# AkshayThiru/incentive-design-mpc

Hardware: AMD Instinct MI355X
Metric: LoMPC QP solves/sec (higher is better)
Workload: dtype f64

## Files before the change

### incentive-design-mpc_amd/csrc/lompc_plan.hip

```cpp
#include <hip/hip_ext.h>
#include <hip/hip_runtime.h>
#include <stdint.h>
#include <string.h>

#include <algorithm>
#include <chrono>
#include <cmath>
#include <cstdlib>
#include <map>
#include <mutex>
#include <type_traits>
#include <utility>

#include "lompc_ctx.hpp"
#include "lompc_loopstep.hpp"
#include "lompc_wave.hpp"

#ifdef LOMPC_STAMPS
#ifdef LOMPC_STAMPS_RT
#define __builtin_amdgcn_s_memtime __builtin_amdgcn_s_memrealtime
#endif
__device__ long long g_stamps[65536 * 8];
__device__ long long g_wstart[32768 * 8];
__device__ unsigned long long g_lstamps[64 * 16];
#define LQ_WSTART()                                                                              \
  do {                                                                                           \
    const long long t__ = __builtin_amdgcn_s_memtime();                                          \
    if ((threadIdx.x & 63) == 0 && blockIdx.x < 32768) g_wstart[blockIdx.x * 8 + (threadIdx.x >> 6)] = t__; \
  } while (0)
#define LQ_STAMPE(k)                                                                        \
  do {                                                                                      \
    const long long t__ = __builtin_amdgcn_s_memtime();                                     \
    if (threadIdx.x == 0 && blockIdx.x < 32768) g_stamps[(32768 + blockIdx.x) * 8 + (k)] = t__; \
  } while (0)
#define LQ_STAMPW(k)                                                                        \
  do {                                                                                      \
    asm volatile("s_waitcnt vmcnt(0)" ::: "memory");                                        \
    LQ_STAMPE(k);                                                                           \
  } while (0)
#define LQ_STAMP(k)                                                                         \
  do {                                                                                      \
    const long long t__ = __builtin_amdgcn_s_memtime();                                     \
    if ((threadIdx.x & 63) == 0 && blk < 65536) g_stamps[blk * 8 + (k)] = t__;              \
  } while (0)
#else
#define LQ_STAMP(k)
#define LQ_STAMPE(k)
#define LQ_STAMPW(k)
#define LQ_WSTART()
#endif

#ifndef EVAL_WAVES
#define EVAL_WAVES 8
#endif
#ifndef EVAL_RU
#define EVAL_RU 2
#endif
#ifndef EVAL_MIN_WAVES
#define EVAL_MIN_WAVES ((2 * EVAL_WAVES + 3) / 4)
#endif
#define EVAL_EVS (64 * EVAL_WAVES)
#ifndef EVAL_PASSES
#define EVAL_PASSES 2
#endif
#define EVAL_MAXB (EVAL_EVS * EVAL_PASSES)
#ifndef LQ_PIECE_CAP
#define LQ_PIECE_CAP 128
#endif
#define LQ_GMAX 1024
#ifndef LQ_EVAL_OUT_AFTER_ROWS
#define LQ_EVAL_OUT_AFTER_ROWS 1
#endif
#ifndef LQ_DIAG_NOLOOKUP
#define LQ_DIAG_NOLOOKUP 0
#endif
#ifndef LQ_DIAG_NOROWLDS
#define LQ_DIAG_NOROWLDS 0
#endif
#ifndef LQ_STEP_CELLS
#define LQ_STEP_CELLS 4
#endif
#ifndef LQ_STEP_PRIO
#define LQ_STEP_PRIO 1
#endif
#ifndef LQ_WARM_FP64
#define LQ_WARM_FP64 1
#endif
#define LQ_DROP_OFF 0x7fff0000

namespace {

typedef unsigned int lq_v4u __attribute__((ext_vector_type(4)));
typedef unsigned int lq_v2u __attribute__((ext_vector_type(2)));

#ifndef LQ_ROW_AUX
#define LQ_ROW_AUX 16
#endif
__device__ __forceinline__ void st_wt16(__amdgpu_buffer_rsrc_t rs, int off, double x, double y) {
  __builtin_amdgcn_raw_buffer_store_b128(__builtin_bit_cast(lq_v4u, make_double2(x, y)), rs, off, 0, LQ_ROW_AUX);
}
__device__ __forceinline__ void st_wt8b(__amdgpu_buffer_rsrc_t rs, int off, double x) {
  __builtin_amdgcn_raw_buffer_store_b64(__builtin_bit_cast(lq_v2u, x), rs, off, 0, LQ_ROW_AUX);
}
__device__ __forceinline__ void st_wt8(double* p, double v) {
  __hip_atomic_store(reinterpret_cast<unsigned long long*>(p), __builtin_bit_cast(unsigned long long, v),
                     __ATOMIC_RELAXED, __HIP_MEMORY_SCOPE_AGENT);
}

#ifndef LQ_EV_PLAIN
#define LQ_EV_PLAIN 0
#endif
__device__ __forceinline__ void st_ev8(double* p, double v) {
  if (LQ_EV_PLAIN) *p = v;
  else st_wt8(p, v);
}

__device__ __forceinline__ void st_wt4(int* p, int v) {
  __hip_atomic_store(p, v, __ATOMIC_RELAXED, __HIP_MEMORY_SCOPE_AGENT);
}

__host__ __device__ constexpr int eval_row_stride(int N) { return N + 1; }
__device__ __forceinline__ int cfx(const int k, const int j) {
  return k * 8 + ((((j >> 1) ^ (k >> 2)) & 3) << 1) + (j & 1);
}
static_assert((LQ_PPL & (LQ_PPL - 1)) == 0, "k_eval's piece-end transpose needs a power-of-two LQ_PPL");

#ifndef LQ_EVALS_STAGER
#define LQ_EVALS_STAGER 0
#endif
#ifndef LQ_EVALS_CAP
#define LQ_EVALS_CAP 64
#endif
#ifndef LQ_STG_CHUNK
#define LQ_STG_CHUNK 8
#endif
#define LQ_EVALS_RW 7
#define LQ_EVALS_MAXB (LQ_EVALS_RW * 64 * EVAL_PASSES)

struct CTab {
  double2* ab;
  double* cf;
  double* ge;
  double* lo;
  int* cnt;
  int* pre;
  int* meta;
};
__host__ __device__ inline size_t ctab_bytes(int N, int G, int capc) {
  const size_t b = (size_t)(capc + 2) * eval_row_stride(N) * 16 + (size_t)capc * 64 + (size_t)(capc + 8) * 8 +
                   (size_t)G * 16 + 16;
  return (b + 15) & ~(size_t)15;
}
__device__ __forceinline__ CTab ctab_at(char* base, int N, int G, int capc) {
  CTab t;
  t.ab = reinterpret_cast<double2*>(base);
  t.cf = reinterpret_cast<double*>(base + (size_t)(capc + 2) * eval_row_stride(N) * 16);
  t.ge = t.cf + (size_t)capc * 8;
  t.lo = t.ge + capc + 8;
  t.cnt = reinterpret_cast<int*>(t.lo + G);
  t.pre = t.cnt + G;
  t.meta = t.pre + G;
  return t;
}
inline size_t evals_st_lds(int N, int G, int capc) {
  return 2 * ctab_bytes(N, G, capc) + (size_t)2 * EVAL_WAVES * (N + 8) * sizeof(double);
}

__device__ __forceinline__ double clampw(double x, double wmax) { return fmin(fmax(x, 0.0), wmax); }

typedef const __attribute__((address_space(4))) QPConst QPConstK;
__device__ __forceinline__ const QPConst& set_consts(const QPConst* qd, const CtxEnds& ce, int s) {
  s = __builtin_amdgcn_readfirstlane(s);
  int k = 0;
#pragma unroll
  for (int j = 0; j + 1 < LQ_PLAN_MAX_CTX; ++j) k += s >= ce.end[j] ? 1 : 0;
  QPConstK* p = (QPConstK*)(uintptr_t)qd + k;
  return *(const QPConst*)p;
}

struct WindowArgs {
  const QPConst* qd;
  CtxEnds ce;
  const int4* blk;
  const int* blk_prefix;
  const double* gamma;
  unsigned long long* acc;
  double* window;
  int S, nblk;
};

__device__ __forceinline__ void window_store(double* window, int s, double ym, bool any, double lo, double hi) {
  const double mg = 1e-7 * ym;
  double wlo = 0.0, whi = ym;
  if (any) {
    wlo = fmin(fmax(lo - mg, 0.0), ym);
    whi = fmin(fmax(hi + mg, wlo + mg), ym);
    if (!(whi > wlo)) wlo = fmax(whi - 2.0 * mg, 0.0);
  }
  window[2 * s] = wlo;
  window[2 * s + 1] = whi;
}

__global__ __launch_bounds__(256) void k_plan_window(WindowArgs a) {
  __shared__ double smin[4], smax[4];
  __shared__ int last;
  if ((int)blockIdx.x == a.nblk) {
    for (int s = threadIdx.x; s < a.S; s += 256)
      if (a.blk_prefix[s + 1] == a.blk_prefix[s]) {
        int k = 0;
        for (int j = 0; j + 1 < LQ_PLAN_MAX_CTX; ++j) k += s >= a.ce.end[j] ? 1 : 0;
        a.window[2 * s] = 0.0;
        a.window[2 * s + 1] = a.qd[k].y_max;
      }
    return;
  }
  const int4 bk = a.blk[blockIdx.x];
// ... 602 lines not shown
    const bool is_max = c >= SN && (c - SN) % LOMPC_SET_STATS == LOMPC_STAT_MAX_ERR;
    double v = recv[c];
    for (int k = 1; k < nranks; ++k) {
      const double x = recv[(size_t)k * L + c];
      v = is_max ? fmax(v, x) : v + x;
    }
    if (c < SN) {
      if (set_sum_w) set_sum_w[c] = v;
    } else if (set_stats) {
      set_stats[c - SN] = v;
    }
  }
}

struct CombineRunsArgs {
  const double* recv;
  int nranks, n, S, N, run0, last;
  double* set_sum_w;
  double* set_stats;
  int64_t sw_stride, st_stride;
};
__global__ __launch_bounds__(256) void k_combine_runs(CombineRunsArgs a) {
  const int SN = a.S * a.N, L = a.S * (a.N + LOMPC_SET_STATS);
  const int64_t tot = (int64_t)a.n * L;
  for (int64_t e = (int64_t)blockIdx.x * 256 + threadIdx.x; e < tot; e += (int64_t)gridDim.x * 256) {
    const int r = (int)(e / L), c = (int)(e - (int64_t)r * L), j = a.run0 + r;
    const bool is_max = c >= SN && (c - SN) % LOMPC_SET_STATS == LOMPC_STAT_MAX_ERR;
    double v = a.recv[(size_t)r * L + c];
    for (int k = 1; k < a.nranks; ++k) {
      const double x = a.recv[((size_t)k * a.n + r) * L + c];
      v = is_max ? fmax(v, x) : v + x;
    }
    if (c < SN) {
      if (a.set_sum_w && (a.sw_stride || j == a.last)) a.set_sum_w[(size_t)j * a.sw_stride + c] = v;
    } else if (a.set_stats && (a.st_stride || j == a.last)) {
      a.set_stats[(size_t)j * a.st_stride + c - SN] = v;
    }
  }
}

__global__ __launch_bounds__(256) void k_chain_price(const QPConst* __restrict__ q, CtxEnds ce, int nctx, int N,
                                                     const double* __restrict__ prev, const double* __restrict__ sum_w,
                                                     const double* __restrict__ stats,
                                                     const double* __restrict__ target, double step,
                                                     double* __restrict__ next) {
  const int s = blockIdx.x;
  int k = 0;
  while (k + 1 < nctx && s >= ce.end[k]) ++k;
  const double th = q[k].theta, wm = q[k].w_max, qs = q[k].q_scale;
  const double n = stats[(size_t)s * LOMPC_SET_STATS + LOMPC_STAT_COUNT];
  for (int i = threadIdx.x; i < 3 * N; i += blockDim.x) {
    const int seg = i / N, t = i - seg * N;
    const double x = prev[(size_t)s * 3 * N + i];
    double v = x;
    if (n > 0) {
      const double wb = sum_w[(size_t)s * N + t] / n, wr = target[(size_t)s * N + t];
      const double g = seg == 0 ? th * (wb - wr) : (seg == 1 ? th * ((wm - wb) - (wm - wr)) : qs * (wb * wb - wr * wr));
      v = fmax(0.0, x + step * g);
    }
    next[(size_t)s * 3 * N + i] = v;
  }
}

struct RunOff {
  int64_t tab = 0;
  int rec = 0;
  int64_t ev = 0;
  const double* lmbd = nullptr;
  const double* lmbd_r = nullptr;
  bool launder = false;
  bool gamma_lds = false;
  bool nostage = false;
  bool pipelined = false;
  bool first = false;
  int buf = 0;
};

__device__ __forceinline__ void stage_compact(const EvalArgs& a, const int s, const int64_t tab, const CTab T,
                                           const int N, const int G, const int capc, const int lane) {
  const int64_t cb = tab + (int64_t)s * G;
  int cn = 0;
  double cl = 0.0;
  if (lane < G) {
    cn = min(max(ld_t<false>(a.t_cnt + cb + lane), 0), LQ_PPL);
    cl = ld_t<false>(a.t_lo + cb + lane);
  }
  int incl = cn;
#pragma unroll
  for (int d = 1; d < 64; d <<= 1) {
    const int y = __shfl_up(incl, d, 64);
    if (lane >= d) incl += y;
  }
  const bool fit = incl <= capc;
  const int ends = fit ? incl : 0x7fffffff;
  const int pre = incl - cn;
  int np = fit ? incl : 0, mx = fit ? cn : 0;
#pragma unroll
  for (int d = 32; d >= 1; d >>= 1) {
    np = max(np, __shfl_xor(np, d, 64));
    mx = max(mx, __shfl_xor(mx, d, 64));
  }
  if (lane < G) {
    T.cnt[lane] = fit ? cn : 0;
    T.pre[lane] = pre;
    T.lo[lane] = cl;
  }
  if (lane == 0) {
    T.meta[0] = mx;
    T.meta[1] = np;
  }
  const int NS = eval_row_stride(N);
  const size_t sb = (size_t)cb * LQ_PPL;
  for (int p0 = 0; p0 < np; p0 += LQ_STG_CHUNK) {
    double2 v[LQ_STG_CHUNK];
    int sl = 0;
#pragma unroll
    for (int u = 0; u < LQ_STG_CHUNK; ++u) {
      const int p = p0 + u;
      const int c = __popcll(__ballot(lane < G && ends <= p));
      const int slot = c * LQ_PPL + p - __builtin_amdgcn_readlane(pre, min(c, 63));
      if (lane == u) sl = slot;
      const double2* src = lane < N ? a.t_ab + (sb + slot) * N + lane
                                    : reinterpret_cast<const double2*>(a.t_cf + (sb + slot) * 8) + (lane - N);
      v[u] = p < np && lane < N + 4 ? ld_t<false>(src) : make_double2(0.0, 0.0);
    }
    const double vg = lane < LQ_STG_CHUNK && p0 + lane < np ? ld_t<false>(a.t_ge + sb + sl) : 0.0;
#pragma unroll
    for (int u = 0; u < LQ_STG_CHUNK; ++u) {
      const int p = p0 + u;
      if (p < np) {
        if (lane < N) T.ab[p * NS + ((N & 1) ? lane : (lane & 1) * (N >> 1) + (lane >> 1))] = v[u];
        else if (lane < N + 4) *reinterpret_cast<double2*>(T.cf + cfx(p, 2 * (lane - N))) = v[u];
      }
    }
    if (lane < LQ_STG_CHUNK && p0 + lane < np) T.ge[p0 + lane] = vg;
  }
}

template <int NT = 0, bool CLOSE = false, bool STG = false>
__device__ __forceinline__ void eval_block(const EvalArgs& a, const int blk, const FinalArgs* fr = nullptr,
                                           const RunOff ro = RunOff{}) {
  static_assert(!(STG && CLOSE), "the staged form has no in-launch closing");
  extern __shared__ __attribute__((aligned(16))) double2 s_dyn[];
  __shared__ double s_g[EVAL_MAXB];
  __shared__ int s_k[EVAL_MAXB];
  __shared__ double s_accw[EVAL_WAVES][LOMPC_MAX_N];
  __shared__ double s_red[EVAL_WAVES][8];
  __shared__ int s_fc[EVAL_WAVES];
  __shared__ int s_last;
  __shared__ int s_mx;
  __shared__ int s_done;
  int tid_ = (int)threadIdx.x;
  if (ro.launder) asm volatile("" : "+v"(tid_));
  const int tid = tid_, lane = tid & 63, wv = tid >> 6;
  const int4 info = a.blk[blk];
  const int rb = ro.rec + blk;
  double* const aw = a.w ? a.w + ro.ev * (NT ? NT : a.N) : nullptr;
  double* const acost = a.cost ? a.cost + ro.ev : nullptr;
  double* const aw0 = a.w0 ? a.w0 + ro.ev : nullptr;
  int8_t* const astatus = a.status ? a.status + ro.ev : nullptr;
  const int s = info.x, start = info.y, end = info.z;
  const int sg_per = STG ? (end - start + LQ_EVALS_RW - 1) / LQ_EVALS_RW : 0;
  const int sg0 = STG ? wv * sg_per : 0;
  const int sgn = STG ? max(0, min(sg_per, end - start - sg0)) : 0;
  auto brow = [&](const int h) { return STG ? sg0 + 64 * h + lane : tid + EVAL_EVS * h; };
  auto bact = [&](const int h) { return STG ? 64 * h + lane < sgn : start + tid + EVAL_EVS * h < end; };
  LQ_STAMPW(6);
  int G_ = a.G, cap_ = a.cap;
  if (ro.launder) asm volatile("" : "+s"(G_), "+s"(cap_));
  const int N = NT ? NT : a.N, G = G_;
  const int cap = cap_;
  const int ZK = cap;
  const int ZD = cap + 1;
  const bool psum = !CLOSE && !STG && ro.pipelined && a.piece_sums && !aw;
  LQ_STAMPE(0);
  LQ_WSTART();
  const int NS = eval_row_stride(N);
  auto abx = [&](const int k, const int t) { return k * NS + ((N & 1) ? t : (t & 1) * (N >> 1) + (t >> 1)); };
  double2* s_ab = s_dyn;
  double* s_cf = reinterpret_cast<double*>(s_ab + (size_t)(cap + 2) * NS);
  double* s_ge = s_cf + (size_t)cap * 8;
  double* s_lo = s_ge + cap;
  int* s_cnt = reinterpret_cast<int*>(s_lo + G);
  int* s_pre = nullptr;
  int stg_meta[2] = {0, 0};
  if constexpr (STG) {
    const CTab T = ctab_at(reinterpret_cast<char*>(s_dyn) + (size_t)ro.buf * ctab_bytes(N, G, cap), N, G, cap);
    s_ab = T.ab;
    s_cf = T.cf;
    s_ge = T.ge;
    s_lo = T.lo;
    s_cnt = T.cnt;
    s_pre = T.pre;
    stg_meta[0] = T.meta[0];
    stg_meta[1] = T.meta[1];
  }
  unsigned long long* s_pf = reinterpret_cast<unsigned long long*>(s_cnt + ((G + 1) & ~1));
  int* s_pn = reinterpret_cast<int*>(s_pf + cap + 2);
  const int np = STG ? stg_meta[1] : min(G * LQ_PPL, cap);
  const int Gs = STG ? G : np / LQ_PPL;
  constexpr int CPW = (LQ_PIECE_CAP / LQ_PPL + EVAL_WAVES - 1) / EVAL_WAVES;
  constexpr int UA = ((NT ? NT : LOMPC_MAX_N) * LQ_PPL + 63) / 64;
  int wc = 0;
  if (!STG && lane < CPW && wv + EVAL_WAVES * lane < Gs)
    wc = ld_t<false>(a.t_cnt + ro.tab + (size_t)s * G + wv + EVAL_WAVES * lane);
  double gh[EVAL_PASSES];
#pragma unroll
  for (int h = 0; h < EVAL_PASSES; ++h) {
    const int i = start + brow(h);
    gh[h] = ro.gamma_lds ? s_g[brow(h)] : bact(h) ? a.gamma[i] : 0.0;
  }
  const QPConst& q = set_consts(a.qd, a.ce, s);
  double wlo = a.window[2 * s], whi = a.window[2 * s + 1];
  const double* __restrict__ L = (ro.lmbd ? ro.lmbd : a.lmbd) + (size_t)s * 3 * N;
  double l0[3] = {L[0], L[N], L[2 * N]};
  double lr = (ro.lmbd_r ? ro.lmbd_r : a.lmbd_r)[s];
  const int64_t cb = ro.tab + (int64_t)s * G;
  const size_t sb = (size_t)cb * LQ_PPL;
  if (ro.pipelined && ro.first && tid == 0) s_done = 0;
  if constexpr (!STG) if (!ro.nostage) {
    int vn = 0;
    double vl = 0.0;
    if (tid < G) {
      vn = ld_t<false>(a.t_cnt + cb + tid);
      vl = ld_t<false>(a.t_lo + cb + tid);
    }
    lq_tab_fill(q);
    lq_pin(wlo);
    lq_pin(whi);
    lq_pin(l0[0]);
    lq_pin(l0[1]);
    lq_pin(l0[2]);
    lq_pin(lr);
    LQ_STAMPW(2);
    double2 v[CPW][UA];
    double vc[CPW], vg[CPW];
    int nc[CPW];
#pragma unroll
    for (int j = 0; j < CPW; ++j)
      nc[j] = min(max(lqw::readlane_i(wc, j), 0), LQ_PPL);
#pragma unroll
    for (int j = 0; j < CPW; ++j) {
      const int c = wv + EVAL_WAVES * j;
      const size_t so = sb + (size_t)c * LQ_PPL;
#pragma unroll
      for (int u = 0; u < UA; ++u) {
        const int it = lane + 64 * u;
        v[j][u] = it < nc[j] * N ? ld_t<false>(a.t_ab + so * N + it) : make_double2(0.0, 0.0);
      }
      vc[j] = lane < nc[j] * 8 ? ld_t<false>(a.t_cf + so * 8 + lane) : 0.0;
      vg[j] = lane < nc[j] ? ld_t<false>(a.t_ge + so + lane) : 0.0;
    }
    LQ_STAMPW(3);
    if (ro.pipelined) __syncthreads();
#pragma unroll
    for (int j = 0; j < CPW; ++j) {
      const int c = wv + EVAL_WAVES * j;
#pragma unroll
      for (int u = 0; u < UA; ++u) {
        const int it = lane + 64 * u;
        if (it < nc[j] * N) {
          const int k = it / N;
          s_ab[abx(c * LQ_PPL + k, it - k * N)] = v[j][u];
        }
      }
      if (lane < nc[j] * 8) s_cf[cfx(c * LQ_PPL + (lane >> 3), lane & 7)] = vc[j];
      if (lane < nc[j]) s_ge[lane * Gs + c] = vg[j];
    }
    if (tid < G) {
      s_cnt[tid] = vn;
      s_lo[tid] = vl;
    }
    if (wv == 0) {
      const double m = lqw::wave_max(tid < G ? (double)vn : 0.0, 64);
      if (lane == 0) s_mx = G <= 64 ? (int)m : LQ_PPL;
    }
    if (tid < 2 * NS) s_ab[ZK * NS + tid] = make_double2(0.0, 0.0);
    if ((CLOSE || psum) && tid < cap + 2) {
      s_pf[tid] = 0ull;
      s_pn[tid] = 0;
    }
    for (int c = tid + EVAL_EVS; c < G; c += EVAL_EVS) {
      s_cnt[c] = ld_t<false>(a.t_cnt + cb + c);
      s_lo[c] = ld_t<false>(a.t_lo + cb + c);
    }
  }
  if constexpr (!STG) __syncthreads();
  LQ_STAMPE(1);
  const double ym = q.y_max, wm = q.w_max;
  const double tt = q.theta * q.theta;
  const double cscale = (double)G / (whi - wlo);
  const double fxs = 0x1p40 / (whi - wlo);
  double acc_cost = 0.0, acc_p0 = 0.0, acc_err = 0.0;
  int n_ok = 0, n_fail = 0, n_inv = 0, nlist = 0;
  bool inv_rows = false;
  const int mxc = STG ? stg_meta[0] : s_mx;
  int pk[EVAL_PASSES];
  unsigned pf[EVAL_PASSES];
  auto lookup_key = [&](const int h) {
    const int i = start + brow(h);
    const bool act = bact(h);
    const double g = gh[h];
    const bool valid = act && g >= 0.0 && g <= ym;
    const int c = valid ? cell_of(g, wlo, cscale, G) : 0;
    const int nc = s_cnt[c];
    const int kb = STG ? s_pre[c] : c * LQ_PPL, ke = kb + nc;
    double ge[LQ_PPL];
#pragma unroll
    for (int k = 0; k < LQ_PPL; ++k)
      ge[k] = (k < mxc && !LQ_DIAG_NOLOOKUP) ? s_ge[STG ? kb + k : k * Gs + min(c, Gs - 1)] : 0.0;
    const double glo_c = s_lo[c];
    int key = kb;
    double gend = ge[0];
#pragma unroll
    for (int k = 0; k + 1 < LQ_PPL; ++k) key += (k + 1 < nc && g > ge[k]) ? 1 : 0;
#pragma unroll
    for (int k = 1; k < LQ_PPL; ++k) gend = nc == k + 1 ? ge[k] : gend;
    const bool cov = LQ_DIAG_NOLOOKUP ? valid && ke > kb
                                      : valid && ke > kb && (STG || ke <= np) && g >= glo_c && g <= gend;
    pk[h] = key;
    pf[h] = (cov ? 1u : 0u) | ((act && !valid) ? 2u : 0u);
    if (!STG || act) {
      s_g[brow(h)] = g;
      s_k[brow(h)] = cov ? key : ((CLOSE && valid) ? ZD : ZK);
    }
    inv_rows |= __ballot(act && !valid) != 0ull;
    const unsigned long long need = __ballot(valid && !cov);
    if (valid && !cov) {
      st_wt4(a.fail_idx + (size_t)rb * EVAL_MAXB + 64 * EVAL_PASSES * wv + nlist +
                 __popcll(need & ((1ull << lane) - 1ull)), i);
      ++n_fail;
    }
    nlist += __popcll(need);
  };
  auto lookup_out = [&](const int h) {
    const int i = start + brow(h);
    const double g = gh[h];
    const int key = pk[h];
    const bool cov = (pf[h] & 1u) != 0u;
    if ((pf[h] & 2u) != 0u) {
      ++n_inv;
      if (acost) st_ev8(acost + i, NAN);
      if (aw0) st_ev8(aw0 + i, NAN);
      if (astatus) astatus[i] = LOMPC_QP_INVALID;
    } else if (cov) {
      const double2 q0 = *reinterpret_cast<const double2*>(s_cf + cfx(key, 0));
      const double2 q1 = *reinterpret_cast<const double2*>(s_cf + cfx(key, 2));
      const double2 q2 = *reinterpret_cast<const double2*>(s_cf + cfx(key, 4));
      const double2 q3 = *reinterpret_cast<const double2*>(s_cf + cfx(key, 6));
      const double4 c0 = make_double4(q0.x, q0.y, q1.x, q1.y), c1 = make_double4(q2.x, q2.y, q3.x, q3.y);
      const double cst = fma(fma(c0.z, g, c0.y), g, c0.x);
      const double e2 = fma(fma(c1.y, g, c1.x), g, c0.w);
      const double er = a.want_err ? fmax(e2, 0.0) : 0.0;
      const double w0v = clampw(fma(c1.w, g, c1.z), wm);
      const double p0 = q.theta * (w0v * l0[0] + (wm - w0v) * l0[1]) + q.q_scale * w0v * w0v * l0[2] +
                        tt * w0v * w0v * lr;
      acc_cost += cst;
      acc_p0 += p0;
      acc_err = fmax(acc_err, er);
      ++n_ok;
      if (acost) st_ev8(acost + i, cst);
      if (aw0) st_ev8(aw0 + i, w0v);
      if (astatus) astatus[i] = LOMPC_QP_OK;
      if (CLOSE || psum) {
        atomicAdd(s_pn + key, 1);
        atomicAdd(s_pf + key, (unsigned long long)rint(fmax(g - wlo, 0.0) * fxs));
      }
    }
  };
  auto lookup = [&](const int h) {
    lookup_key(h);
    lookup_out(h);
  };
  auto pass_live = [&](const int h) { return STG ? 64 * h < sgn : h == 0 || start + EVAL_EVS * h + 64 * wv < end; };
  if constexpr (CLOSE) {
#pragma unroll
    for (int h = 0; h < EVAL_PASSES; ++h)
      if (pass_live(h)) lookup(h);
  }
  LQ_STAMPE(7);
  double* accw_all;
  double* red_all;
  int astr;
  if constexpr (STG) {
    double* scr = reinterpret_cast<double*>(reinterpret_cast<char*>(s_dyn) + 2 * ctab_bytes(N, G, cap));
    accw_all = scr + (size_t)ro.buf * EVAL_WAVES * N;
    red_all = scr + (size_t)2 * EVAL_WAVES * N + (size_t)ro.buf * EVAL_WAVES * 8;
    astr = N;
  } else {
    accw_all = &s_accw[0][0];
    red_all = &s_red[0][0];
    astr = LOMPC_MAX_N;
  }
  double* const red_w = red_all + wv * 8;
  double* const accw_w = accw_all + wv * astr;
  auto wave_record = [&]() {
    double tot[4] = {acc_cost, acc_p0, (double)n_ok, 0.0};
    lqw::wave_totals(tot, 64);
    const double mx = sqrt(lqw::wave_max(acc_err, 64));
    double cnt[2] = {(double)n_fail, (double)n_inv};
    lqw::wave_totals(cnt, 64);
    if (lane == 0) {
      red_w[PX_COST] = tot[0];
      red_w[PX_PRICE0] = tot[1];
      red_w[PX_MAX_ERR] = mx;
      red_w[PX_N_OK] = tot[2];
      red_w[PX_N_REPAIRED] = tot[3];
      red_w[PX_N_FAILED] = cnt[0];
      red_w[PX_N_INVALID] = cnt[1];
    }
  };
  auto store_record = [&](int t, int nthreads) {
    double* part = a.partial + (size_t)rb * (N + NPX);
    for (int c = t; c < N + NPX; c += nthreads) {
      double v = 0.0;
      if (c < N) {
        for (int k = 0; k < EVAL_WAVES; ++k) v += accw_all[k * astr + c];
      } else {
        const int x = c - N;
        for (int k = 0; k < EVAL_WAVES; ++k) v = x == PX_MAX_ERR ? fmax(v, red_all[k * 8 + x]) : v + red_all[k * 8 + x];
      }
      st_wt8(part + c, v);
    }
  };
  bool any_inv = inv_rows;
  if constexpr (CLOSE) {
    if (lane == 0) s_fc[wv] = nlist;
    if (nlist > 0) asm volatile("s_waitcnt vmcnt(0)" ::: "memory");
    __syncthreads();
    const double fxi = (whi - wlo) * 0x1p-40;
    double accs = 0.0;
    constexpr int PU = (LQ_PIECE_CAP + EVAL_WAVES - 1) / EVAL_WAVES;
    for (int p0 = wv; p0 < np; p0 += EVAL_WAVES * PU) {
      int n[PU];
      unsigned long long f[PU];
      double2 ab[PU];
#pragma unroll
      for (int k = 0; k < PU; ++k) {
        const int p = p0 + EVAL_WAVES * k;
        const int pc = min(p, np - 1);
        n[k] = p < np ? s_pn[pc] : 0;
        f[k] = s_pf[pc];
        ab[k] = s_ab[abx(pc, min(lane, N - 1))];
      }
#pragma unroll
      for (int k = 0; k < PU; ++k) {
        const double gsum = fma((double)f[k], fxi, (double)n[k] * wlo);
        accs = fma((double)n[k], n[k] ? ab[k].x : 0.0, accs);
        accs = fma(n[k] ? gsum : 0.0, n[k] ? ab[k].y : 0.0, accs);
      }
    }
    if (lane < N) s_accw[wv][lane] = accs;
    wave_record();
    __syncthreads();
    any_inv = false;
    for (int k = 0; k < EVAL_WAVES; ++k) any_inv |= s_red[k][PX_N_INVALID] > 0.0;
    if (wv == 0) {
      store_record(lane, 64);
      if (lane < EVAL_WAVES) st_wt4(a.fail_cnt + (size_t)rb * EVAL_WAVES + lane, s_fc[lane]);
      asm volatile("s_waitcnt vmcnt(0)" ::: "memory");
      if (lane == 0) {
        const int nb = fr->blk_prefix[s + 1] - fr->blk_prefix[s];
        const int old = __hip_atomic_fetch_add(fr->arrive + s, 1, __ATOMIC_RELAXED, __HIP_MEMORY_SCOPE_AGENT);
        s_last = old == nb - 1;
        if (old == nb - 1) __hip_atomic_store(fr->arrive + s, 0, __ATOMIC_RELAXED, __HIP_MEMORY_SCOPE_AGENT);
      }
    }
  }
  const int V = (N & 1) ? 1 : 2;
  const int Lr = N / V;
  const int R = 64 / Lr;
  const int rr = lane / Lr, col = lane - rr * Lr;
  const bool rlane = rr < R;
  const int t0 = V * col;
  constexpr int RU = EVAL_RU;
  double acc0 = 0.0, acc1 = 0.0;
  const bool fast = aw && a.w_rsrc_ok;
  const __amdgpu_buffer_rsrc_t rs =
      __builtin_amdgcn_make_buffer_rsrc(aw, (short)0, aw ? a.w_bytes : 0, 0x00020000);
  auto row_segment = [&](const int r0b, const int nrows) {
    const int* sk = s_k + r0b;
    const double* sg = s_g + r0b;
    const int rbase = start + r0b;
    const int vb = rlane ? ((rbase + rr) * N + t0) * 8 : LQ_DROP_OFF;
    int kk[RU];
    double gg[RU];
#pragma unroll
    for (int j = 0; j < RU; ++j) {
      const int rc = min(j * R + rr, nrows - 1);
      kk[j] = sk[rc];
      gg[j] = sg[rc];
    }
    for (int r0 = 0; r0 < nrows; r0 += RU * R) {
      double2 u0[RU], u1[RU];
#pragma unroll
      for (int j = 0; j < RU; ++j) {
        if (LQ_DIAG_NOROWLDS) {
          u0[j] = make_double2(1e-3 * kk[j], 1e-3);
          u1[j] = make_double2(2e-3 * kk[j], 1e-3);
        } else {
          u0[j] = s_ab[kk[j] * NS + col];
          u1[j] = V == 2 ? s_ab[kk[j] * NS + (N >> 1) + col] : make_double2(0.0, 0.0);
        }
      }
      int kn[RU];
      double gn[RU];
#pragma unroll
      for (int j = 0; j < RU; ++j) {
        const int rc = min(r0 + (RU + j) * R + rr, nrows - 1);
        kn[j] = sk[rc];
        gn[j] = sg[rc];
      }
      auto rows = [&](auto full_t, auto fast_t) {
        constexpr bool FULL = decltype(full_t)::value, FAST = decltype(fast_t)::value;
#pragma unroll
        for (int j = 0; j < RU; ++j) {
          const double x0 = clampw(fma(u0[j].y, gg[j], u0[j].x), wm);
          const double x1 = V == 2 ? clampw(fma(u1[j].y, gg[j], u1[j].x), wm) : 0.0;
          if (FULL || (rlane && r0 + j * R + rr < nrows && (!CLOSE || kk[j] != ZD))) {
            if (!CLOSE) {
              acc0 += x0;
              acc1 += x1;
            }
            if (FAST) {
              const int off = vb + (r0 + j * R) * N * 8;
              if (V == 2) st_wt16(rs, off, x0, x1);
              else st_wt8b(rs, off, x0);
            } else if (aw) {
              double* dst = aw + (size_t)(rbase + r0 + j * R + rr) * N + t0;
              st_wt8(dst, x0);
              if (V == 2) st_wt8(dst + 1, x1);
            }
          }
        }
      };
      using T_ = std::true_type;
      using F_ = std::false_type;
      bool full = r0 + RU * R <= nrows;
      if constexpr (CLOSE) {
        bool drop = false;
#pragma unroll
        for (int j = 0; j < RU; ++j) drop |= kk[j] == ZD;
        full = full && !__any(drop);
      }
      if (full) {
        if (fast) rows(T_{}, T_{});
        else rows(T_{}, F_{});
      } else {
        if (fast) rows(F_{}, T_{});
        else rows(F_{}, F_{});
      }
#pragma unroll
      for (int j = 0; j < RU; ++j) {
        kk[j] = kn[j];
        gg[j] = gn[j];
      }
    }
    if (any_inv && aw) {
      asm volatile("s_waitcnt vmcnt(0)" ::: "memory");
      for (int r = 0; r < nrows; ++r) {
        const double g = sg[r];
        if (!(g >= 0.0 && g <= ym) && lane < N) st_wt8(aw + (size_t)(rbase + r) * N + lane, NAN);
      }
    }
  };
  if constexpr (CLOSE) {
    if (wv > 0 && aw) {
      const int tot = end - start;
      const int lo = (wv - 1) * tot / (EVAL_WAVES - 1), hi = wv * tot / (EVAL_WAVES - 1);
      if (hi > lo) row_segment(lo, hi - lo);
    }
  } else {
#pragma unroll
    for (int h = 0; h < EVAL_PASSES; ++h) {
      if (!pass_live(h)) break;
      if (LQ_EVAL_OUT_AFTER_ROWS) lookup_key(h);
      else lookup(h);
      __builtin_amdgcn_wave_barrier();
      any_inv = inv_rows;
      const int r0b = STG ? sg0 + 64 * h : EVAL_EVS * h + 64 * wv;
      const int nh = STG ? min(64, sgn - 64 * h) : max(0, min(64, end - start - r0b));
      if (nh > 0 && !psum) row_segment(r0b, nh);
      if (LQ_EVAL_OUT_AFTER_ROWS) lookup_out(h);
    }
    if (lane == 0) st_wt4(a.fail_cnt + (size_t)rb * EVAL_WAVES + wv, nlist);
    wave_record();
  }
  LQ_STAMPE(4);
  if constexpr (CLOSE) {
    __syncthreads();
    if (s_last) {
      double (*red)[FIN_W] = reinterpret_cast<double (*)[FIN_W]>(s_dyn);
      finalize_set<EVAL_WAVES, true>(*fr, s, red, red + EVAL_WAVES);
    }
  } else {
    if (!rlane) acc0 = acc1 = 0.0;
    {
      double s0 = acc0, s1 = acc1;
      for (int k = 1; k < R; ++k) {
        s0 += __shfl(acc0, lane + k * Lr, 64);
        s1 += __shfl(acc1, lane + k * Lr, 64);
      }
      if (lane < Lr) {
        accw_w[V * lane] = s0;
        if (V == 2) accw_w[V * lane + 1] = s1;
      }
    }
    if constexpr (!STG) {
      if (ro.pipelined) {
        int old = 0;
        __builtin_amdgcn_fence(__ATOMIC_RELEASE, "workgroup", "local");
        if (lane == 0) old = __hip_atomic_fetch_add(&s_done, 1, __ATOMIC_ACQ_REL, __HIP_MEMORY_SCOPE_WORKGROUP);
        old = __shfl(old, 0, 64);
        __builtin_amdgcn_fence(__ATOMIC_ACQUIRE, "workgroup", "local");
        if (old == EVAL_WAVES - 1) {
          if (psum) {
            const double fxi = (whi - wlo) * 0x1p-40;
            double accs = 0.0;
            for (int p = 0; p < np; ++p) {
              const int n = s_pn[p];
              if (n == 0) continue;
              const double2 ab = s_ab[abx(p, min(lane, N - 1))];
              const double gsum = fma((double)s_pf[p], fxi, (double)n * wlo);
              accs = fma((double)n, ab.x, accs);
              accs = fma(gsum, ab.y, accs);
            }
            if (lane < N) accw_w[lane] = accs;
            __builtin_amdgcn_fence(__ATOMIC_RELEASE, "wavefront");
          }
          store_record(lane, 64);
          if (lane == 0) __hip_atomic_store(&s_done, 0, __ATOMIC_RELAXED, __HIP_MEMORY_SCOPE_WORKGROUP);
        }
      } else {
        __syncthreads();
        if (tid < 64) store_record(tid, 64);
      }
    }
  }
  LQ_STAMPE(5);
}

template <bool CLOSE, int NT>
__global__ __launch_bounds__(EVAL_EVS, EVAL_MIN_WAVES) void k_eval(EvalArgs a, FinalArgs r) {
  extern __shared__ __attribute__((aligned(16))) double2 s_dyn[];
  const int b = (int)blockIdx.x;
  if (a.skip && *a.skip) return;
  if constexpr (CLOSE) {
    if (b == a.nblk) {
      double (*red)[FIN_W] = reinterpret_cast<double (*)[FIN_W]>(s_dyn);
      for (int s = 0; s < a.S; ++s)
        if (r.blk_prefix[s + 1] == r.blk_prefix[s]) {
          finalize_set<EVAL_WAVES, true>(r, s, red, red + EVAL_WAVES);
          __syncthreads();
        }
      return;
    }
  }
  eval_block<NT, CLOSE>(a, b, &r);
}

typedef void (*EvalKernel)(EvalArgs, FinalArgs);
template <bool CLOSE>
EvalKernel eval_kernel(int N) {
  switch (N) {
    case 12: return k_eval<CLOSE, 12>;
    case 16: return k_eval<CLOSE, 16>;
    case 24: return k_eval<CLOSE, 24>;
    case 48: return k_eval<CLOSE, 48>;
    default: return k_eval<CLOSE, 0>;
  }
}

template <int NT>
__global__ __launch_bounds__(EVAL_EVS, EVAL_MIN_WAVES) void k_step(PathArgs pa, EvalArgs ea, FinalArgs ff, int np_wg,
                                                                    int ne, int nf) {
  extern __shared__ __attribute__((aligned(16))) double2 s_dyn[];
  int b = (int)blockIdx.x;
  if (b < np_wg) {
    const int wv = (int)(threadIdx.x >> 6), cell = b * LQ_STEP_CELLS + wv;
    if (wv >= LQ_STEP_CELLS || cell >= pa.S * pa.G) return;
    if (LQ_STEP_PRIO) __builtin_amdgcn_s_setprio(3);
    path_cell<NT, true>(pa, cell);
    return;
  }
  b -= np_wg;
  if (b < ne) {
    eval_block<NT, false>(ea, b);
    return;
  }
  b -= ne;
  if (b < nf) {
    double (*red)[FIN_W] = reinterpret_cast<double (*)[FIN_W]>(s_dyn);
    finalize_set<EVAL_WAVES, false>(ff, b, red, red + EVAL_WAVES);
  }
}

typedef void (*StepKernel)(PathArgs, EvalArgs, FinalArgs, int, int, int);
StepKernel step_kernel(int N) {
  switch (N) {
    case 12: return k_step<12>;
    case 16: return k_step<16>;
    case 24: return k_step<24>;
    case 48: return k_step<48>;
    default: return k_step<0>;
  }
}

#ifndef LQ_PATHS_WAVES
#define LQ_PATHS_WAVES 1
#endif
template <int NT>
__global__ __launch_bounds__(64, LQ_PATHS_WAVES) void k_paths(PathArgs a, int64_t lm_stride, int64_t lr_stride, int run0,
                                                               int slots) {
  const int SG = a.S * a.G;
  const int r = (int)blockIdx.x / SG, cell = (int)blockIdx.x - r * SG;
  const int j = run0 + r;
  const int64_t o = (int64_t)(j % slots) * SG;
  PathArgs b = a;
  b.lmbd = a.lmbd + (size_t)j * lm_stride;
  b.lmbd_r = a.lmbd_r + (size_t)j * lr_stride;
  b.t_cnt = a.t_cnt + o;
  b.t_lo = a.t_lo + o;
  b.t_sl = a.t_sl + o * 64;
  b.t_ge = a.t_ge + o * LQ_PPL;
  b.t_cf = a.t_cf + o * LQ_PPL * 8;
  b.t_ab = a.t_ab + o * LQ_PPL * a.N;
  path_cell<NT, true>(b, cell);
}

typedef void (*PathsKernel)(PathArgs, int64_t, int64_t, int, int);
PathsKernel paths_kernel(int N) {
  switch (N) {
    case 12: return k_paths<12>;
    case 16: return k_paths<16>;
    case 24: return k_paths<24>;
    case 48: return k_paths<48>;
    default: return k_paths<0>;
  }
}

struct EvalsArgs {
  int run0, nruns, slots, nblk;
  int64_t lm_stride, lr_stride, ev_stride, SG;
};

#ifndef LQ_EVALS_PIPELINED
#define LQ_EVALS_PIPELINED 1
#endif
#ifndef LQ_EVALS_RUN_BARRIER
#define LQ_EVALS_RUN_BARRIER 0
#endif
#ifndef LQ_EVALS_SKEW
#define LQ_EVALS_SKEW 0
#endif

template <int NT>
__global__ __launch_bounds__(EVAL_EVS, EVAL_MIN_WAVES) void k_evals(EvalArgs a, EvalsArgs x) {
  const int b = (int)blockIdx.x;
  if (LQ_EVALS_SKEW > 0 && 2 * b >= x.nblk) {
    const long long t0 = __builtin_amdgcn_s_memrealtime();
    while (__builtin_amdgcn_s_memrealtime() - t0 < LQ_EVALS_SKEW) __builtin_amdgcn_s_sleep(8);
  }
  for (int r = 0; r < x.nruns; ++r) {
    const int j = x.run0 + r;
    RunOff ro;
    ro.tab = (int64_t)(j % x.slots) * x.SG;
    ro.rec = r * x.nblk;
    ro.ev = (int64_t)j * x.ev_stride;
    ro.lmbd = a.lmbd + (size_t)j * x.lm_stride;
    ro.lmbd_r = a.lmbd_r + (size_t)j * x.lr_stride;
    ro.launder = true;
    ro.gamma_lds = r > 0;
    ro.pipelined = LQ_EVALS_PIPELINED;
    ro.first = r == 0;
#ifdef LQ_EVALS_NOSTAGE
    ro.nostage = r > 0;
#endif
    int bl = b;
    asm volatile("" : "+s"(bl));
#ifdef LOMPC_STAMPS
    const long long t0__ = __builtin_amdgcn_s_memtime();
#endif
    eval_block<NT, false>(a, bl, nullptr, ro);
#if LQ_EVALS_RUN_BARRIER
    __syncthreads();
#endif
#ifdef LOMPC_STAMPS
    if (threadIdx.x == 0 && r < 32 && b < 512) {
      long long* q = g_stamps + ((size_t)b * 32 + r) * 8;
      const long long* e = g_stamps + (32768 + b) * 8;
      q[0] = t0__;
      q[1] = e[6];
      q[2] = e[0];
      q[3] = e[2];
      q[4] = e[3];
      q[5] = e[1];
      q[6] = e[4];
      q[7] = __builtin_amdgcn_s_memtime();
    }
#endif
  }
}

template <int NT>
__global__ __launch_bounds__(EVAL_EVS, EVAL_MIN_WAVES) void k_evals_st(EvalArgs a, EvalsArgs x) {
  extern __shared__ __attribute__((aligned(16))) double2 s_dyn[];
  const int b = (int)blockIdx.x, tid = (int)threadIdx.x, lane = tid & 63;
  const int wv = __builtin_amdgcn_readfirstlane(tid >> 6);
  const int N = NT ? NT : a.N, G = a.G, capc = a.cap;
  const size_t tb = ctab_bytes(N, G, capc);
  char* const base = reinterpret_cast<char*>(s_dyn);
  double* const accw = reinterpret_cast<double*>(base + 2 * tb);
  double* const red = accw + (size_t)2 * EVAL_WAVES * N;
  const int s = a.blk[b].x;
  if (wv == LQ_EVALS_RW) {
    const int NS = eval_row_stride(N);
    for (int k = 0; k < 2; ++k) {
      const CTab T = ctab_at(base + k * tb, N, G, capc);
      for (int i = lane; i < 2 * NS; i += 64) T.ab[(size_t)capc * NS + i] = make_double2(0.0, 0.0);
      for (int i = lane; i < N; i += 64) accw[((size_t)k * EVAL_WAVES + LQ_EVALS_RW) * N + i] = 0.0;
      if (lane < 8) red[((size_t)k * EVAL_WAVES + LQ_EVALS_RW) * 8 + lane] = 0.0;
    }
    stage_compact(a, s, (int64_t)(x.run0 % x.slots) * x.SG, ctab_at(base, N, G, capc), N, G, capc, lane);
  }
  __syncthreads();
  for (int r = 0; r < x.nruns; ++r) {
    const int j = x.run0 + r;
    if (wv < LQ_EVALS_RW) {
      RunOff ro;
      ro.tab = (int64_t)(j % x.slots) * x.SG;
      ro.rec = r * x.nblk;
      ro.ev = (int64_t)j * x.ev_stride;
      ro.lmbd = a.lmbd + (size_t)j * x.lm_stride;
      ro.lmbd_r = a.lmbd_r + (size_t)j * x.lr_stride;
      ro.launder = true;
      ro.gamma_lds = r > 0;
      ro.buf = r & 1;
      int bl = b;
      asm volatile("" : "+s"(bl));
      eval_block<NT, false, true>(a, bl, nullptr, ro);
    } else if (r + 1 < x.nruns) {
      stage_compact(a, s, (int64_t)((j + 1) % x.slots) * x.SG, ctab_at(base + ((r + 1) & 1) * tb, N, G, capc), N, G,
                    capc, lane);
    }
    __syncthreads();
    if (wv == 0) {
      const int rb = r * x.nblk + b;
      const int par = r & 1;
      double* part = a.partial + (size_t)rb * (N + NPX);
      for (int c = lane; c < N + NPX; c += 64) {
        double v = 0.0;
        if (c < N) {
          for (int k = 0; k < EVAL_WAVES; ++k) v += accw[((size_t)par * EVAL_WAVES + k) * N + c];
        } else {
          const int xx = c - N;
          for (int k = 0; k < EVAL_WAVES; ++k) {
            const double u = red[((size_t)par * EVAL_WAVES + k) * 8 + xx];
            v = xx == PX_MAX_ERR ? fmax(v, u) : v + u;
          }
        }
        st_wt8(part + c, v);
      }
      if (lane == 0) st_wt4(a.fail_cnt + (size_t)rb * EVAL_WAVES + LQ_EVALS_RW, 0);
    }
  }
}

typedef void (*EvalsKernel)(EvalArgs, EvalsArgs);
EvalsKernel evals_st_kernel(int N) {
  switch (N) {
    case 12: return k_evals_st<12>;
    case 16: return k_evals_st<16>;
    case 24: return k_evals_st<24>;
    case 48: return k_evals_st<48>;
    default: return k_evals_st<0>;
  }
}
EvalsKernel evals_kernel(int N) {
  switch (N) {
    case 12: return k_evals<12>;
    case 16: return k_evals<16>;
    case 24: return k_evals<24>;
    case 48: return k_evals<48>;
    default: return k_evals<0>;
  }
}

struct ClosesArgs {
  int run0, nruns, slots, nblk, S, last;
  int rel;
  int64_t lm_stride, lr_stride, ev_stride, sw_stride, st_stride, SG;
};

__global__ __launch_bounds__(256) void k_closes(FinalArgs f, ClosesArgs x) {
  __shared__ double red[LQ_FIN_CLASSES][FIN_W];
  __shared__ double rep[LQ_FIN_CLASSES][FIN_W];
  const int r = (int)blockIdx.x / x.S, s = (int)blockIdx.x - r * x.S, j = x.run0 + r, N = f.N;
  FinalArgs c = f;
  c.lmbd = f.lmbd + (size_t)j * x.lm_stride;
  c.lmbd_r = f.lmbd_r + (size_t)j * x.lr_stride;
  c.t_sl = f.t_sl + (int64_t)(j % x.slots) * x.SG * 64;
  c.partial = f.partial + (size_t)r * x.nblk * (N + NPX);
  c.fail_cnt = f.fail_cnt + (size_t)r * x.nblk * EVAL_WAVES;
  c.fail_idx = f.fail_idx + (size_t)r * x.nblk * EVAL_MAXB;
  const bool last = j == x.last;
  if (x.ev_stride) {
    const size_t eo = (size_t)j * x.ev_stride;
    if (f.w) c.w = f.w + eo * N;
    if (f.cost) c.cost = f.cost + eo;
    if (f.w0) c.w0 = f.w0 + eo;
    if (f.status) c.status = f.status + eo;
  } else if (!last) {
    c.w = c.cost = c.w0 = nullptr;
    c.status = nullptr;
  }
  const int js = x.rel ? r : j;
  if (f.set_sum_w) c.set_sum_w = (x.sw_stride || last) ? f.set_sum_w + (size_t)js * x.sw_stride : nullptr;
  if (f.set_stats) c.set_stats = (x.st_stride || last) ? f.set_stats + (size_t)js * x.st_stride : nullptr;
  if (!last) c.stats = nullptr;
  finalize_set<4, false>(c, s, red, rep);
}

#include "lompc_agg.hpp"

constexpr int LQ_LOOP_G = 16;
constexpr int LQ_LOOP_G2 = 32;

#ifdef LOMPC_STAMPS
#define LQ_LSTAMP(k)                                                                                 \
  do {                                                                                               \
    asm volatile("s_waitcnt vmcnt(0)" ::: "memory");                                                 \
    const long long t__ = __builtin_amdgcn_s_memrealtime();                                          \
    if (lane == 0 && blk < 64) {                                                                     \
      __hip_atomic_fetch_add(g_lstamps + blk * 16 + (k), (unsigned long long)(t__ - tl__), __ATOMIC_RELAXED, \
                             __HIP_MEMORY_SCOPE_AGENT);                                              \
      if ((k) == 0 || (k) == 3 || (k) == 4)                                                          \
// ... 1797 lines not shown
```

Measured before the change: 20.94 billion.

## Scalarize wave-uniform values, specialize lookup by piece count, read kernargs directly

Makes the wave index and row counts scalar via readfirstlane, and specializes the piece lookup on the per-block max piece count so the compare loops shrink. Wave counters now use ballot/popcount instead of per-lane increments and cross-lane reductions, and the max-error reduction is skipped when errors are not requested. Row batches are split into a full-batch loop plus a tail so the full/fast branch is chosen once. Kernel arguments are re-read from the kernarg segment each run to cut register pressure. The aim is fewer VGPRs and less per-row overhead, at the cost of more code size from the added specializations.

```diff
diff --git a/incentive-design-mpc_amd/csrc/lompc_plan.hip b/incentive-design-mpc_amd/csrc/lompc_plan.hip
--- a/incentive-design-mpc_amd/csrc/lompc_plan.hip
+++ b/incentive-design-mpc_amd/csrc/lompc_plan.hip
@@ -62,6 +62,12 @@
 #define EVAL_EVS (64 * EVAL_WAVES)
 #ifndef EVAL_PASSES
 #define EVAL_PASSES 2
+#endif
+#ifndef LQ_EVAL_WV_SCALAR
+#define LQ_EVAL_WV_SCALAR 1
+#endif
+#ifndef LQ_EVALS_KARGS
+#define LQ_EVALS_KARGS 1
 #endif
 #define EVAL_MAXB (EVAL_EVS * EVAL_PASSES)
 #ifndef LQ_PIECE_CAP
@@ -970,7 +976,7 @@
   __shared__ int s_done;
   int tid_ = (int)threadIdx.x;
   if (ro.launder) asm volatile("" : "+v"(tid_));
-  const int tid = tid_, lane = tid & 63, wv = tid >> 6;
+  const int tid = tid_, lane = tid & 63, wv = LQ_EVAL_WV_SCALAR ? __builtin_amdgcn_readfirstlane(tid >> 6) : tid >> 6;
   const int4 info = a.blk[blk];
   const int rb = ro.rec + blk;
   double* const aw = a.w ? a.w + ro.ev * (NT ? NT : a.N) : nullptr;
@@ -1105,17 +1111,18 @@
   }
   if constexpr (!STG) __syncthreads();
   LQ_STAMPE(1);
-  const double ym = q.y_max, wm = q.w_max;
+  const double ym = q.y_max, wm = __builtin_canonicalize(q.w_max);
   const double tt = q.theta * q.theta;
   const double cscale = (double)G / (whi - wlo);
   const double fxs = 0x1p40 / (whi - wlo);
   double acc_cost = 0.0, acc_p0 = 0.0, acc_err = 0.0;
-  int n_ok = 0, n_fail = 0, n_inv = 0, nlist = 0;
+  int n_ok = 0, n_inv = 0, nlist = 0;
   bool inv_rows = false;
   const int mxc = STG ? stg_meta[0] : s_mx;
   int pk[EVAL_PASSES];
   unsigned pf[EVAL_PASSES];
-  auto lookup_key = [&](const int h) {
+  auto lookup_key_mx = [&](auto mx_t, const int h) {
+    constexpr int MX = decltype(mx_t)::value, KE = MX ? MX : LQ_PPL;
     const int i = start + brow(h);
     const bool act = bact(h);
     const double g = gh[h];
@@ -1125,15 +1132,15 @@
     const int kb = STG ? s_pre[c] : c * LQ_PPL, ke = kb + nc;
     double ge[LQ_PPL];
 #pragma unroll
-    for (int k = 0; k < LQ_PPL; ++k)
-      ge[k] = (k < mxc && !LQ_DIAG_NOLOOKUP) ? s_ge[STG ? kb + k : k * Gs + min(c, Gs - 1)] : 0.0;
+    for (int k = 0; k < KE; ++k)
+      ge[k] = ((MX || k < mxc) && !LQ_DIAG_NOLOOKUP) ? s_ge[STG ? kb + k : k * Gs + min(c, Gs - 1)] : 0.0;
     const double glo_c = s_lo[c];
     int key = kb;
     double gend = ge[0];
 #pragma unroll
-    for (int k = 0; k + 1 < LQ_PPL; ++k) key += (k + 1 < nc && g > ge[k]) ? 1 : 0;
-#pragma unroll
-    for (int k = 1; k < LQ_PPL; ++k) gend = nc == k + 1 ? ge[k] : gend;
+    for (int k = 0; k + 1 < KE; ++k) key += (k + 1 < nc && g > ge[k]) ? 1 : 0;
+#pragma unroll
+    for (int k = 1; k < KE; ++k) gend = nc == k + 1 ? ge[k] : gend;
     const bool cov = LQ_DIAG_NOLOOKUP ? valid && ke > kb
                                       : valid && ke > kb && (STG || ke <= np) && g >= glo_c && g <= gend;
     pk[h] = key;
@@ -1147,17 +1154,27 @@
     if (valid && !cov) {
       st_wt4(a.fail_idx + (size_t)rb * EVAL_MAXB + 64 * EVAL_PASSES * wv + nlist +
                  __popcll(need & ((1ull << lane) - 1ull)), i);
-      ++n_fail;
     }
     nlist += __popcll(need);
+  };
+  const int mxu = __builtin_amdgcn_readfirstlane(mxc);
+  auto lookup_key = [&](const int h) {
+    switch (mxu) {
+      case 1: lookup_key_mx(std::integral_constant<int, 1>{}, h); break;
+      case 2: lookup_key_mx(std::integral_constant<int, 2>{}, h); break;
+      case 3: lookup_key_mx(std::integral_constant<int, 3>{}, h); break;
+      case 4: lookup_key_mx(std::integral_constant<int, 4>{}, h); break;
+      default: lookup_key_mx(std::integral_constant<int, 0>{}, h); break;
+    }
   };
   auto lookup_out = [&](const int h) {
     const int i = start + brow(h);
     const double g = gh[h];
     const int key = pk[h];
     const bool cov = (pf[h] & 1u) != 0u;
+    n_inv += __popcll(__ballot((pf[h] & 2u) != 0u));
+    n_ok += __popcll(__ballot(pf[h] == 1u));
     if ((pf[h] & 2u) != 0u) {
-      ++n_inv;
       if (acost) st_ev8(acost + i, NAN);
       if (aw0) st_ev8(aw0 + i, NAN);
       if (astatus) astatus[i] = LOMPC_QP_INVALID;
@@ -1176,7 +1193,6 @@
       acc_cost += cst;
       acc_p0 += p0;
       acc_err = fmax(acc_err, er);
-      ++n_ok;
       if (acost) st_ev8(acost + i, cst);
       if (aw0) st_ev8(aw0 + i, w0v);
       if (astatus) astatus[i] = LOMPC_QP_OK;
@@ -1213,19 +1229,17 @@
   double* const red_w = red_all + wv * 8;
   double* const accw_w = accw_all + wv * astr;
   auto wave_record = [&]() {
-    double tot[4] = {acc_cost, acc_p0, (double)n_ok, 0.0};
+    double tot[2] = {acc_cost, acc_p0};
     lqw::wave_totals(tot, 64);
-    const double mx = sqrt(lqw::wave_max(acc_err, 64));
-    double cnt[2] = {(double)n_fail, (double)n_inv};
-    lqw::wave_totals(cnt, 64);
+    const double mx = a.want_err ? sqrt(lqw::wave_max(acc_err, 64)) : 0.0;
     if (lane == 0) {
       red_w[PX_COST] = tot[0];
       red_w[PX_PRICE0] = tot[1];
       red_w[PX_MAX_ERR] = mx;
-      red_w[PX_N_OK] = tot[2];
-      red_w[PX_N_REPAIRED] = tot[3];
-      red_w[PX_N_FAILED] = cnt[0];
-      red_w[PX_N_INVALID] = cnt[1];
+      red_w[PX_N_OK] = (double)n_ok;
+      red_w[PX_N_REPAIRED] = 0.0;
+      red_w[PX_N_FAILED] = (double)nlist;
+      red_w[PX_N_INVALID] = (double)n_inv;
     }
   };
   auto store_record = [&](int t, int nthreads) {
@@ -1296,9 +1310,14 @@
   const bool fast = aw && a.w_rsrc_ok;
   const __amdgpu_buffer_rsrc_t rs =
       __builtin_amdgcn_make_buffer_rsrc(aw, (short)0, aw ? a.w_bytes : 0, 0x00020000);
+  typedef double lds_d2v __attribute__((ext_vector_type(2)));
+  typedef __attribute__((address_space(3))) const lds_d2v lds_cd2;
+  typedef __attribute__((address_space(3))) const double lds_cd;
+  typedef __attribute__((address_space(3))) const int lds_ci;
   auto row_segment = [&](const int r0b, const int nrows) {
-    const int* sk = s_k + r0b;
-    const double* sg = s_g + r0b;
+    lds_ci* sk = (lds_ci*)(s_k + r0b);
+    lds_cd* sg = (lds_cd*)(s_g + r0b);
+    lds_cd2* sab = (lds_cd2*)s_ab;
     const int rbase = start + r0b;
     const int vb = rlane ? ((rbase + rr) * N + t0) * 8 : LQ_DROP_OFF;
     int kk[RU];
@@ -1309,28 +1328,33 @@
       kk[j] = sk[rc];
       gg[j] = sg[rc];
     }
-    for (int r0 = 0; r0 < nrows; r0 += RU * R) {
-      double2 u0[RU], u1[RU];
-#pragma unroll
-      for (int j = 0; j < RU; ++j) {
-        if (LQ_DIAG_NOROWLDS) {
-          u0[j] = make_double2(1e-3 * kk[j], 1e-3);
-          u1[j] = make_double2(2e-3 * kk[j], 1e-3);
-        } else {
-          u0[j] = s_ab[kk[j] * NS + col];
-          u1[j] = V == 2 ? s_ab[kk[j] * NS + (N >> 1) + col] : make_double2(0.0, 0.0);
+    auto batches = [&](auto full_t, auto fast_t, const int rb, const int re) {
+      constexpr bool FULL = decltype(full_t)::value, FAST = decltype(fast_t)::value;
+      for (int r0 = rb; r0 < re; r0 += RU * R) {
+        double2 u0[RU], u1[RU];
+#pragma unroll
+        for (int j = 0; j < RU; ++j) {
+          if (LQ_DIAG_NOROWLDS) {
+            u0[j] = make_double2(1e-3 * kk[j], 1e-3);
+            u1[j] = make_double2(2e-3 * kk[j], 1e-3);
+          } else {
+            const lds_d2v p0 = sab[kk[j] * NS + col];
+            u0[j] = make_double2(p0.x, p0.y);
+            u1[j] = make_double2(0.0, 0.0);
+            if (V == 2) {
+              const lds_d2v p1 = sab[kk[j] * NS + (N >> 1) + col];
+              u1[j] = make_double2(p1.x, p1.y);
+            }
+          }
         }
-      }
-      int kn[RU];
-      double gn[RU];
-#pragma unroll
-      for (int j = 0; j < RU; ++j) {
-        const int rc = min(r0 + (RU + j) * R + rr, nrows - 1);
-        kn[j] = sk[rc];
-        gn[j] = sg[rc];
-      }
-      auto rows = [&](auto full_t, auto fast_t) {
-        constexpr bool FULL = decltype(full_t)::value, FAST = decltype(fast_t)::value;
+        int kn[RU];
+        double gn[RU];
+#pragma unroll
+        for (int j = 0; j < RU; ++j) {
+          const int rc = min(r0 + (RU + j) * R + rr, nrows - 1);
+          kn[j] = sk[rc];
+          gn[j] = sg[rc];
+        }
 #pragma unroll
         for (int j = 0; j < RU; ++j) {
           const double x0 = clampw(fma(u0[j].y, gg[j], u0[j].x), wm);
@@ -1351,27 +1375,37 @@
             }
           }
         }
-      };
-      using T_ = std::true_type;
-      using F_ = std::false_type;
-      bool full = r0 + RU * R <= nrows;
-      if constexpr (CLOSE) {
+#pragma unroll
+        for (int j = 0; j < RU; ++j) {
+          kk[j] = kn[j];
+          gg[j] = gn[j];
+        }
+      }
+    };
+    using T_ = std::true_type;
+    using F_ = std::false_type;
+    if constexpr (CLOSE) {
+      for (int r0 = 0; r0 < nrows; r0 += RU * R) {
         bool drop = false;
 #pragma unroll
         for (int j = 0; j < RU; ++j) drop |= kk[j] == ZD;
-        full = full && !__any(drop);
-      }
-      if (full) {
-        if (fast) rows(T_{}, T_{});
-        else rows(T_{}, F_{});
+        const bool full = r0 + RU * R <= nrows && !__any(drop);
+        if (full) {
+          if (fast) batches(T_{}, T_{}, r0, r0 + 1);
+          else batches(T_{}, F_{}, r0, r0 + 1);
+        } else {
+          if (fast) batches(F_{}, T_{}, r0, r0 + 1);
+          else batches(F_{}, F_{}, r0, r0 + 1);
+        }
+      }
+    } else {
+      const int nfull = nrows - nrows % (RU * R);
+      if (fast) {
+        batches(T_{}, T_{}, 0, nfull);
+        if (nfull < nrows) batches(F_{}, T_{}, nfull, nrows);
       } else {
-        if (fast) rows(F_{}, T_{});
-        else rows(F_{}, F_{});
-      }
-#pragma unroll
-      for (int j = 0; j < RU; ++j) {
-        kk[j] = kn[j];
-        gg[j] = gn[j];
+        batches(T_{}, F_{}, 0, nfull);
+        if (nfull < nrows) batches(F_{}, F_{}, nfull, nrows);
       }
     }
     if (any_inv && aw) {
@@ -1397,7 +1431,7 @@
       __builtin_amdgcn_wave_barrier();
       any_inv = inv_rows;
       const int r0b = STG ? sg0 + 64 * h : EVAL_EVS * h + 64 * wv;
-      const int nh = STG ? min(64, sgn - 64 * h) : max(0, min(64, end - start - r0b));
+      const int nh = __builtin_amdgcn_readfirstlane(STG ? min(64, sgn - 64 * h) : max(0, min(64, end - start - r0b)));
       if (nh > 0 && !psum) row_segment(r0b, nh);
       if (LQ_EVAL_OUT_AFTER_ROWS) lookup_out(h);
     }
@@ -1572,21 +1606,36 @@
 #define LQ_EVALS_SKEW 0
 #endif
 
+constexpr size_t KARG_X = (sizeof(EvalArgs) + alignof(EvalsArgs) - 1) / alignof(EvalsArgs) * alignof(EvalsArgs);
+static_assert(alignof(EvalArgs) <= 8 && alignof(EvalsArgs) <= 8, "k_evals reads its arguments at offsets 0 and KARG_X");
+
 template <int NT>
-__global__ __launch_bounds__(EVAL_EVS, EVAL_MIN_WAVES) void k_evals(EvalArgs a, EvalsArgs x) {
+__global__ __launch_bounds__(EVAL_EVS, EVAL_MIN_WAVES) void k_evals(EvalArgs a, EvalsArgs x_) {
   const int b = (int)blockIdx.x;
-  if (LQ_EVALS_SKEW > 0 && 2 * b >= x.nblk) {
+  if (LQ_EVALS_SKEW > 0 && 2 * b >= x_.nblk) {
     const long long t0 = __builtin_amdgcn_s_memrealtime();
     while (__builtin_amdgcn_s_memrealtime() - t0 < LQ_EVALS_SKEW) __builtin_amdgcn_s_sleep(8);
   }
-  for (int r = 0; r < x.nruns; ++r) {
+  for (int r = 0; r < x_.nruns; ++r) {
+#if LQ_EVALS_KARGS
+    typedef __attribute__((address_space(4))) const EvalArgs karg_t;
+    typedef __attribute__((address_space(4))) const EvalsArgs kargx_t;
+    typedef __attribute__((address_space(4))) const char kargc_t;
+    karg_t* ka = (karg_t*)__builtin_amdgcn_kernarg_segment_ptr();
+    asm volatile("" : "+s"(ka));
+    const EvalArgs& ar = *(const EvalArgs*)ka;
+    const EvalsArgs& x = *(const EvalsArgs*)(kargx_t*)((kargc_t*)ka + KARG_X);
+#else
+    const EvalArgs& ar = a;
+    const EvalsArgs& x = x_;
+#endif
     const int j = x.run0 + r;
     RunOff ro;
     ro.tab = (int64_t)(j % x.slots) * x.SG;
     ro.rec = r * x.nblk;
     ro.ev = (int64_t)j * x.ev_stride;
-    ro.lmbd = a.lmbd + (size_t)j * x.lm_stride;
-    ro.lmbd_r = a.lmbd_r + (size_t)j * x.lr_stride;
+    ro.lmbd = ar.lmbd + (size_t)j * x.lm_stride;
+    ro.lmbd_r = ar.lmbd_r + (size_t)j * x.lr_stride;
     ro.launder = true;
     ro.gamma_lds = r > 0;
     ro.pipelined = LQ_EVALS_PIPELINED;
@@ -1599,7 +1648,7 @@
 #ifdef LOMPC_STAMPS
     const long long t0__ = __builtin_amdgcn_s_memtime();
 #endif
-    eval_block<NT, false>(a, bl, nullptr, ro);
+    eval_block<NT, false>(ar, bl, nullptr, ro);
 #if LQ_EVALS_RUN_BARRIER
     __syncthreads();
 #endif
```

Result: faster. 23.72 billion (median of 6 runs) (+13.2%).
